# angelini/raft-simulation

Hardware: AMD Instinct MI355X
Metric: simulated node-ticks/sec (5-node Raft) (higher is better)
Workload: dtype u32; 1 GPU; C2: 65,536 5-node clusters/GPU, 10k ticks/step, no faults, no client (steady window); clusters=65536, clusters_per_gpu=65536, nodes=5, parallelism=cluster-sharded x1

## Files before the change

raft-simulation_amd/csrc/fixed_point_affine.hpp:

```cpp
#pragma once
#include <stdint.h>

#if defined(__HIPCC__)
#define FPA_FN __host__ __device__ inline __attribute__((always_inline))
#else
#define FPA_FN inline
#endif

namespace rs {
namespace fpa {

constexpr uint64_t M = 0x9E3779B97F4A7C15ull;
constexpr uint64_t M2 = M * M;
constexpr uint32_t EV_HEARTBEAT = 7, EV_APPEND_ENTRIES = 2, EV_APPEND_RESPONSE = 5;
constexpr uint32_t ROLE_LEADER = 2, ROLE_FOLLWER = 3;
constexpr uint32_t HDR_HB = EV_HEARTBEAT | ROLE_LEADER << 7;
constexpr uint32_t HDR_AR = EV_APPEND_RESPONSE | ROLE_LEADER << 7;
constexpr uint32_t HDR_AE = EV_APPEND_ENTRIES | ROLE_FOLLWER << 7;

constexpr uint64_t pow_m2(int n) {
  uint64_t x = 1;
  for (int i = 0; i < n; ++i) x *= M2;
  return x;
}
// ... 65 lines not shown
  r.z = g.a * f.z + g.z + kp * g.x;
  r.s = (uint32_t)g.a * f.s + g.s;
  return r;
}
FPA_FN Set compose(const Set& f, const Set& g, uint32_t P) {
  const uint64_t kp = (uint64_t)f.K * P;
  Set r;
  r.K = f.K + g.K;
  r.lead = compose_half(f.lead, g.lead, kp);
  r.fol = compose_half(f.fol, g.fol, kp);
  return r;
}

FPA_FN uint32_t period(int F, uint32_t d, uint32_t hb) { return 2 * d + (uint32_t)F - 1 + hb; }

template <int F>
FPA_FN Set step(const Set& c, uint32_t d, uint32_t hb) {
  return compose(c, one_round<F>(d), period(F, d, hb));
}

template <int F>
FPA_FN Set build(uint32_t d, uint32_t hb, uint32_t K) {
  const uint32_t P = period(F, d, hb);
  Set r;
  r.K = 0;
  r.lead.a = r.fol.a = 1;
  r.lead.x = r.lead.y = r.lead.z = r.fol.x = r.fol.y = r.fol.z = 0;
  r.lead.s = r.fol.s = 0;
  if (!K) return r;
  r = one_round<F>(d);
// ... 47 lines not shown
```

raft-simulation_amd/csrc/steady_kernel.hip:

```cpp
#include <hip/hip_ext.h>

#include "fixed_point_affine.hpp"
#include "tick_wave.hpp"

namespace rs {

constexpr int LANE_WG = 256;

__device__ __forceinline__ uint32_t msel(bool a, uint32_t x, uint32_t y) {
  const uint32_t m = 0u - (uint32_t)a;
  return (x & m) | (y & ~m);
}

constexpr int IMG_SLOTS = 32;
constexpr uint32_t IMG_LINE = 64 * 8 * 16;
constexpr uint32_t IMG_HALF = 2 * IMG_LINE;
constexpr uint32_t IMG_WAVE = 2 * IMG_HALF;
__device__ __forceinline__ uint32_t img_sw(uint32_t l) { return (l ^ (l >> 3)) & 7u; }
__device__ __forceinline__ uint32_t img_off(uint32_t l, uint32_t i) {
  return i < 16 ? (i >> 3) * IMG_LINE + l * 128u + 16u * ((i & 7u) ^ img_sw(l))
                : IMG_HALF + l * 256u + 16u * ((i & 15u) ^ (l & 15u));
}
template <typename T>
__device__ __forceinline__ T* lds_at(char* img, uint32_t off) {
// ... 38 lines not shown
  SetWords k[2];
};
__device__ __forceinline__ uint32_t vreg(uint32_t s) {
  uint32_t v;
  asm volatile("v_mov_b32 %0, %1" : "=v"(v) : "s"(s));
  return v;
}
__device__ __forceinline__ uint64_t vreg(uint64_t s) {
  return (uint64_t)vreg((uint32_t)(s >> 32)) << 32 | vreg((uint32_t)s);
}
__device__ __forceinline__ SetWords vreg(const fpa::Set& c, uint32_t K1) {
  return SetWords{vreg(c.lead.a), vreg(c.lead.x), vreg(c.lead.y), vreg(c.lead.z),
                  vreg(c.fol.a),  vreg(c.fol.x),  vreg(c.fol.y),  vreg(c.fol.z),
                  vreg(c.lead.s), vreg(c.fol.s),  vreg(c.K),      vreg(K1)};
}
template <int F>
__device__ __forceinline__ void band_sets(uint32_t nt, uint32_t d, uint32_t hb, BandSets* out) {
  const uint32_t P = fpa::period(F, d, hb), last = 2 * d + F - 1;
  const uint32_t K1 = nt > last ? (nt - last - 1) / P + 1 : 0;
  const fpa::Set lo = fpa::build<F>(d, hb, K1 ? K1 - 1 : 0), hi = fpa::step<F>(lo, d, hb);
  out->k[0] = vreg(lo, K1);
  out->k[1] = vreg(hi, K1);
}

template <int N>
struct FixedPoint {
  static constexpr int F = N - 1;
  uint32_t L, Lid, Lterm, Lcommit;
  uint64_t Ltr, ftr[F];
  uint32_t Ldl, fdl[F], fpend;
  uint32_t qmask, qA[F], qT[F], qa[F], qb[F];
  uint32_t rmask, resA, rT[F], rA[F], rB[F], rH[F];
  uint32_t nhb, nae, nar;

  __device__ __forceinline__ uint32_t fk(int j) const { return (uint32_t)j + ((uint32_t)j >= L ? 1u : 0u); }

  __device__ __forceinline__ void append_entries(uint32_t ta, uint32_t d, uint32_t el_base) {
#pragma unroll
    for (int j = 0; j < F; ++j) {
      ftr[j] = trace_event(ftr[j], ta, RAFT_MSG_APPEND_ENTRIES, Lid, Lterm, RAFT_FOLLWER, Lterm, 0);
      fdl[j] = ta + el_base;
      rT[j] = Lterm; rA[j] = Lcommit; rB[j] = 0; rH[j] = 1;
// ... 78 lines not shown
#pragma unroll
    for (int j = 0; j < F; ++j) {
      if (on && ((rmask >> j) & 1)) {
        uint4* dp = rp + 2 * n;
        dp[0] = make_uint4(resA, RAFT_MSG_APPEND_RESPONSE | sid(j) << 3 | rH[j] << 7, rT[j], rA[j]);
        dp[1] = make_uint4(rB[j], 0, 0, 0);
        ++n;
      }
    }
  }
};

template <int N>
struct NodeOrder {
  static constexpr int F = N - 1;
  uint32_t L, T;
  uint64_t tr[N], Ltr;
  uint32_t Ldl;
  bool qin, took;
  uint32_t qA, fdl;
  uint32_t rc, resA;
  uint32_t nhb, nae, nar;

  __device__ __forceinline__ uint32_t sid(int j) const {
    return (uint32_t)j + 1 + ((uint32_t)j >= L ? 1u : 0u);
  }
  __device__ __forceinline__ void followers(uint64_t a, uint64_t add) {
#pragma unroll
    for (int k = 0; k < N; ++k) tr[k] = tr[k] * a + add;
  }
// ... 13 lines not shown
      if ((uint32_t)j + rc >= (uint32_t)F && tau < tend) {
        Ltr = trace_event(Ltr, tau, RAFT_MSG_APPEND_RESPONSE, sid(j), T, RAFT_LEADER, T, 0);
        --rc;
        Ldl = tau + hb;
        ++nar;
      }
    }
    if (!rc) resA = INF;
  }
  __device__ __forceinline__ uint32_t term() const { return T; }
  __device__ __forceinline__ void rearmed(uint32_t v) { took = true; fdl = v; }
  __device__ __forceinline__ void heartbeat(uint32_t ta) { qin = true; qA = ta; }
  __device__ __forceinline__ bool queued() const { return rc != 0; }
};

template <typename St>
__device__ __forceinline__ void rounds(St& s, uint32_t th, uint32_t tend, uint32_t d, uint32_t hb,
                                       uint32_t el_base, const BandSets& bs) {
  constexpr int F = St::F;
  const uint32_t P = 2 * d + F - 1 + hb, last = 2 * d + F - 1, T = s.term();
  const uint32_t K = tend > th + last ? (tend - th - last - 1) / P + 1 : 0;
  const uint32_t tk = th + K * P;
  if (K) {
    const uint32_t K1 = bs.k[0].K1;
    const bool top = K == K1;
    if (!__builtin_amdgcn_ballot_w64(!top && K + 1 != K1)) {
      const SetWords sw = bs.k[top];
      const fpa::Half cl = sw.lead(), cf = sw.fol();
      s.Ltr = fpa::apply_leader<F>(cl, s.Ltr, th, T, s.L);
      s.followers(cf.a, fpa::follower_addend<F>(cf, th, T, s.L));
    } else {
      uint64_t a = trace_term(th, 7, 0, 0, RAFT_LEADER, T, 0);
#pragma unroll
      for (int j = 0; j < F; ++j)
        a = a * TRACE_M2 + trace_term(th + 2 * d + j, RAFT_MSG_APPEND_RESPONSE, s.sid(j), T,
                                      RAFT_LEADER, T, 0);
      const uint64_t da = (uint64_t)P * (TRACE_M * trace_geo<F + 1>());
      const uint64_t df = (uint64_t)P * TRACE_M;
// ... 14 lines not shown
  if (tk < tend) {
    s.Ltr = trace_event(s.Ltr, tk, 7, 0, 0, RAFT_LEADER, T, 0);
    ++s.nhb;
    s.Ldl = tk + hb;
    s.heartbeat(tk + d);
    if (tk + d < tend) {
      s.append_entries(tk + d, d, el_base);
      s.responses(tk, tend, d, hb);
    }
  }
}

template <typename St>
__device__ __forceinline__ void run_launch(St& s, uint32_t mid, uint32_t th0, uint32_t tend,
                                           uint32_t d, uint32_t hb, uint32_t el_base, uint32_t P,
                                           const BandSets& bs) {
  bool whole = true;
  if (mid == 1) {
    if (th0 + d < tend) s.append_entries(th0 + d, d, el_base);
    else whole = false;
  }
  if (mid && whole) {
    s.responses(th0, tend, d, hb);
    whole = !s.queued();
  }
  if (whole) rounds(s, mid ? th0 + P : th0, tend, d, hb, el_base, bs);
}

struct Schedule {
  uint32_t mid, th0, nxt;
  bool on;
};
template <int F>
__device__ __forceinline__ Schedule schedule(uint32_t t0, uint32_t tend, uint32_t d, uint32_t hb,
                                             uint32_t P, uint32_t Ldl, bool req, uint32_t reqA,
                                             uint32_t nres, uint32_t resA) {
  Schedule s{0, Ldl, 0, true};
  if (req) {
    s.mid = 1;
    s.th0 = reqA - d;
    s.on = reqA >= t0 && reqA >= d && Ldl == s.th0 + hb;
// ... 106 lines not shown
  };
  auto fword = [&](int f, int j, uint32_t L) {
    return msel((uint32_t)j >= L, word(f, j + 1), word(f, j));
  };
  static_assert(HF_RES_TAIL + 1 == HF_FLAGS && (HOT_CW + HF_FLAGS * N) % 4 == 0 && HOT_CW % 4 == 0,
                "the fields written: DEADLINE .. RES_TAIL, whole chunks");
  constexpr int CH_END = (int)(HOT_CW + HF_FLAGS * N) / 4;
  asm volatile("" ::"s"(nt), "s"(t0), "s"(S.dmin), "s"(S.hb), "s"(S.el_base));
  load_line(0, false);
  const bool reporter = blockIdx.x == 0 && threadIdx.x == 0;
  uint32_t prev_bails = 0;
  if (reporter) prev_bails = *S.nbail_zero;
  uint32_t nt_s = nt;
  asm volatile("" : "+s"(nt_s));
  const BandSets& bs = bs_keep[wave];
  band_sets<F>(nt_s, S.dmin, S.hb, &bs_keep[wave]);
  load_wait();
  if (reporter && prev_bails) {
    if (S.bail_report) *S.bail_report = prev_bails;
    *S.nbail_zero = 0;
  }
  static_assert(NW4 >= 8, "line 0 is read whole");
  read_chunks(0, 8);
  const uint32_t tend = t0 + nt, d = S.dmin;
  const uint32_t P = 2 * d + F - 1 + S.hb, allF = (1u << F) - 1;
  uint32_t dl = 0, nhb = 0, nae = 0, nar = 0;
  bool el = false;
  uint32_t el_to = 0;
#ifdef RS_WAVELOG
  uint64_t wl_x1 = 0, wl_x2 = 0, wl_x3 = 0, wl_lend = 0;
  uint32_t wl_cut = 0;
  asm volatile("" ::"v"(w[CL_CERT]), "v"(w[HOT_CW]));
  wl_loop = wall_clock64();
#endif

  static_assert(HOT_CW + (HF_QMETA + 1) * N <= 32 && HF_DEADLINE < HF_QMETA &&
                    HF_TRACE_LO < HF_QMETA && HF_TRACE_HI < HF_QMETA && CL_CTERM < HOT_CW,
                "every word the line-0 path reads is in line 0; REQ_ARR, RES_ARR, the flags and "
                "the term are derived (device.hpp)");
  NodeOrder<N> no;
  uint32_t lmid = 0, lth0 = 0;
  const bool cfg_ok = S.el_base >= P && S.hb >= 2 * d + F && S.Q >= (uint32_t)F;
  bool strong = active && cfg_ok && (w[CL_CERT] & 0xFFFF0000u) == CERT_STRONG &&
                (w[CL_CERT] & 0xFFFFu) < (uint32_t)N;
  {
    const uint32_t L = w[CL_CERT] & 0xFFFFu;
    no.L = L; no.T = w[CL_CTERM];
    no.Ldl = lword(HF_DEADLINE, L);
    no.Ltr = (uint64_t)lword(HF_TRACE_HI, L) << 32 | lword(HF_TRACE_LO, L);
#pragma unroll
    for (int k = 0; k < N; ++k) no.tr[k] = (uint64_t)word(HF_TRACE_HI, k) << 32 | word(HF_TRACE_LO, k);
    no.qin = no.took = false; no.qA = no.fdl = 0; no.rc = 0; no.resA = INF;
    no.nhb = no.nae = no.nar = 0;
    const uint32_t Lqm = lword(HF_QMETA, L), rsc = qm_res_cnt(Lqm);
    const uint32_t qm0 = L ? word(HF_QMETA, 0) : word(HF_QMETA, 1);
    const bool need = qm0 != 0;
    strong = strong && (qm0 & ~pack_qmeta(0, 1, 0, 0)) == 0 && Lqm == pack_qmeta(0, 0, 0, rsc) &&
             rsc <= (uint32_t)F && !(need && rsc);
#pragma unroll
    for (int k = 0; k < N; ++k) strong = strong && (L == (uint32_t)k || word(HF_QMETA, k) == qm0);
    lth0 = no.Ldl;
    if (need) {
      lmid = 1;
      lth0 = no.Ldl - S.hb;
      const uint32_t ta = lth0 + d;
      strong = strong && no.Ldl >= S.hb && ta >= t0;
      no.qin = true;
      no.qA = ta;
    } else if (rsc) {
      lmid = 2;
      const uint32_t j0 = (uint32_t)F - rsc, back = S.hb + (j0 ? 2 * d + j0 - 1 : 0u);
      lth0 = no.Ldl - back;
      const uint32_t ra = lth0 + 2 * d;
      const int64_t cut = (int64_t)t0 - (int64_t)ra;
      strong = strong && no.Ldl >= back &&
               (int64_t)j0 == (cut < 0 ? 0 : cut > F ? (int64_t)F : cut);
      no.rc = rsc;
      no.resA = ra;
    } else {
      strong = strong && no.Ldl >= t0;
    }
    const uint32_t nxt = min((lmid == 2 ? lth0 + P : lth0) + d, tend);
#pragma unroll
    for (int k = 0; k < N; ++k)
      strong = strong && (L == (uint32_t)k || word(HF_DEADLINE, k) >= nxt);
  }
  const bool line0_wave = !__builtin_amdgcn_ballot_w64(active && !strong);
  if (line0_wave) {
#ifdef RS_WAVELOG
    asm volatile("" ::"v"(no.Ltr), "v"(no.Ldl), "v"(no.tr[0]), "v"(lth0));
    wl_x1 = wl_x2 = wall_clock64();
#endif
    if (active) {
      run_launch(no, lmid, lth0, tend, d, S.hb, S.el_base, P, bs);
      nhb = no.nhb; nae = no.nae; nar = no.nar;
#ifdef RS_WAVELOG
      asm volatile("" ::"v"(no.Ltr), "v"(no.tr[0]), "v"(no.Ldl));
      wl_x3 = wall_clock64();
#endif
      const uint32_t fqm = pack_qmeta(0, no.qin ? 1u : 0u, 0, 0), Lqm = pack_qmeta(0, 0, 0, no.rc);
      const uint32_t fra = no.qin ? no.qA : INF, frt = no.qin ? no.qA : 0u;
      const uint32_t Lrt = no.rc ? no.resA : 0u;
      auto val = [&](int q) -> uint32_t {
        const int f = (q - (int)HOT_CW) / N, k = (q - (int)HOT_CW) % N;
        const bool isL = no.L == (uint32_t)k;
        switch (f) {
          case HF_DEADLINE: return isL ? no.Ldl : no.took ? no.fdl : w[q];
          case HF_TRACE_LO: return (uint32_t)(isL ? no.Ltr : no.tr[k]);
          case HF_TRACE_HI: return (uint32_t)((isL ? no.Ltr : no.tr[k]) >> 32);
          case HF_QMETA: return isL ? Lqm : fqm;
          case HF_REQ_ARR: return isL ? INF : fra;
          case HF_RES_ARR: return isL ? no.resA : INF;
          case HF_REQ_TAIL: return isL ? 0u : frt;
          default: return isL ? Lrt : 0u;
        }
      };
      auto chunk = [&](int i) {
        return make_uint4(val(4 * i), val(4 * i + 1), val(4 * i + 2), val(4 * i + 3));
      };
#pragma unroll
      for (int i = (int)HOT_CW / 4; i < (CH_END < 8 ? CH_END : 8); ++i) {
        const int q = 4 * i;
        const uint4 x = chunk(i);
        *lds_at<uint4>(img, img_off(lane, i)) = x;
        dl |= (uint32_t)(x.x != w[q] || x.y != w[q + 1] || x.z != w[q + 2] || x.w != w[q + 3]);
      }
      if (CH_END > 8 && (lmid || no.qin || no.rc)) {
        uint4* const bp = reinterpret_cast<uint4*>(S.hot + (size_t)c * HB);
#pragma unroll
        for (int i = 8; i < CH_END; ++i) bp[i] = chunk(i);
      }
    }
    if (__builtin_amdgcn_ballot_w64(active && (no.qin || no.rc))) {
      if (active && no.qin) {
#pragma unroll
        for (int k = 0; k < N; ++k) {
          if (no.L != (uint32_t)k) {
            uint4* dp = reinterpret_cast<uint4*>(qslots(S, c * N + k, 0));
            dp[0] = make_uint4(no.qA, RAFT_MSG_APPEND_ENTRIES | (no.L + 1) << 3, no.T, 0);
            dp[1] = make_uint4(0, 0, 0, 0);
          }
// ... 31 lines not shown
      Lc = lead ? (uint32_t)k : Lc;
      nlc += lead;
    }
    static_assert(HOT_CW + (HF_FLAGS + 1) * N <= 64, "the flags are in the first two lines");
    cert = active && nlc == 1 &&
           (w[CL_CERT] == (CERT_MAGIC | Lc) || w[CL_CERT] == (CERT_STRONG | Lc));
    full = IMGC > 16 && __builtin_amdgcn_ballot_w64(active && !cert) != 0;
    if (full) {
      load_half1();
      read_chunks(16, NW4);
    }
  }
  const bool vouched = cert && !full;

  FixedPoint<N> fx;
  bool lean = false;
  if (!line0_wave) {
    lean = vouched && cfg_ok;
    const uint32_t L = Lc;
    fx.L = L; fx.Lid = L + 1; fx.Lterm = lword(HF_TERM, L); fx.Lcommit = 0;
    fx.Ldl = lword(HF_DEADLINE, L);
    fx.Ltr = (uint64_t)lword(HF_TRACE_HI, L) << 32 | lword(HF_TRACE_LO, L);
    fx.qmask = fx.rmask = 0; fx.resA = INF; fx.fpend = allF; fx.nhb = fx.nae = fx.nar = 0;
    const uint32_t Lqm = lword(HF_QMETA, L);
    const uint32_t rsc = qm_res_cnt(Lqm);
    uint32_t need = 0;
#pragma unroll
    for (int j = 0; j < F; ++j) {
      fx.fdl[j] = fword(HF_DEADLINE, j, L);
      fx.ftr[j] = (uint64_t)fword(HF_TRACE_HI, j, L) << 32 | fword(HF_TRACE_LO, j, L);
      const uint32_t qm = fword(HF_QMETA, j, L);
      lean = lean && (fword(HF_FLAGS, j, L) & FL_DRAW) && ((qm >> 4) & 31) <= 1 && !qm_res_cnt(qm);
      need |= (qm_req_cnt(qm) ? 1u : 0u) << j;
      fx.qA[j] = INF; fx.qT[j] = fx.qa[j] = fx.qb[j] = 0;
      fx.rT[j] = fx.rA[j] = fx.rB[j] = fx.rH[j] = 0;
    }
    lean = lean && !qm_req_cnt(Lqm) && rsc <= (uint32_t)F && !(need && rsc) &&
           (need == 0 || need == allF);
    const uint32_t ta = fword(HF_REQ_ARR, 0, L), ra = lword(HF_RES_ARR, L);
    const Schedule sc = schedule<F>(t0, tend, d, S.hb, P, fx.Ldl, need != 0, ta, rsc, ra);
    lean = lean && sc.on;
    lmid = sc.mid;
    lth0 = sc.th0;
    if (lmid == 1) {
#pragma unroll
      for (int j = 0; j < F; ++j) {
        lean = lean && fword(HF_REQ_ARR, j, L) == ta;
        fx.qA[j] = ta; fx.qT[j] = fx.Lterm;
      }
      fx.qmask = allF;
    } else if (lmid == 2) {
      fx.rmask = allF & ~((1u << ((uint32_t)F - rsc)) - 1);
      fx.resA = ra;
#pragma unroll
      for (int j = 0; j < F; ++j) {
        fx.rT[j] = fx.Lterm; fx.rH[j] = 1;
      }
    }
#pragma unroll
    for (int j = 0; j < F; ++j) lean = lean && fx.fdl[j] >= sc.nxt;
  }
  const bool lean_wave = !line0_wave && !__builtin_amdgcn_ballot_w64(active && !lean);
  bool wb = false;
  if (lean_wave) {
#ifdef RS_WAVELOG
    asm volatile("" ::"v"(fx.Ltr), "v"(fx.fdl[0]), "v"(fx.ftr[0]), "v"(lth0));
    wl_x1 = wl_x2 = wall_clock64();
#endif
    if (active) {
      run_launch(fx, lmid, lth0, tend, d, S.hb, S.el_base, P, bs);
      nhb = fx.nhb; nae = fx.nae; nar = fx.nar;
#ifdef RS_WAVELOG
      asm volatile("" ::"v"(fx.Ltr), "v"(fx.ftr[0]), "v"(fx.Ldl));
      wl_x3 = wall_clock64();
#endif
      uint32_t v[HF_FLAGS][N];
#pragma unroll
      for (int k = 0; k < N; ++k) fx.node_words(k, v);
      auto val = [&](int q) { return v[(q - HOT_CW) / N][(q - HOT_CW) % N]; };
      auto chunk = [&](int i) {
        return make_uint4(val(4 * i), val(4 * i + 1), val(4 * i + 2), val(4 * i + 3));
      };
#pragma unroll
      for (int i = (int)HOT_CW / 4; i < CH_END; ++i) {
        const int q = 4 * i;
// ... 6 lines not shown
      *lds_at<uint4>(img, img_off(lane, CL_CERT / 4)) =
          make_uint4(w[CL_CERT - 3], w[CL_CERT - 2], fx.Lterm, cn);
      static_assert(CL_CTERM == CL_CERT - 1 && CL_CERT % 4 == 3, "one chunk");
      dl |= (uint32_t)(cn != w[CL_CERT] || fx.Lterm != w[CL_CTERM]);
    }
    fx.to_rings(S, c, active);
#ifdef RS_WAVELOG
    wl_lend = wall_clock64();
#endif
  } else if (!line0_wave) {
#ifdef RS_WAVELOG
    wl_loop = wall_clock64();
#endif
    {
      auto ifield = [&](int f, int k) { return w[HOT_CW + f * N + k]; };
      bool pat = active && w[CL_HWM_IDX] == 0 && S.Q >= 2u * F && S.el_base >= P && S.hb >= 2 * d + F;
      const uint32_t T = ifield(HF_TERM, 0);
#pragma unroll
      for (int k = 0; k < N; ++k) {
        pat = pat && ifield(HF_FLAGS, k) == 0 && ifield(HF_MASKS, k) == 0 &&
              ifield(HF_TERM, k) == T && ifield(HF_COMMIT, k) == 0 && ifield(HF_LEN, k) == 0 &&
              ifield(HF_QMETA, k) == 0 && ifield(HF_REQ_ARR, k) == INF &&
              ifield(HF_RES_ARR, k) == INF;
#pragma unroll
        for (int p = 0; p < 2 * N; ++p) pat = pat && ifield(HF_NEXT + p, k) == 0;
      }
      pat = pat && T != INF;
      uint32_t cidx = 0, t1 = INF, ntie = 0, bidx = 0;
#pragma unroll
      for (int k = 0; k < N; ++k) {
        const uint32_t dk = ifield(HF_DEADLINE, k);
// ... 44 lines not shown
          const uint32_t sid = (uint32_t)j + ((uint32_t)j >= cidx ? 2u : 1u);
          hc = trace_event(hc, (uint32_t)tau0 + j, RAFT_MSG_APPEND_RESPONSE, sid, T, RAFT_LEADER,
                           T1, 0);
        }
#pragma unroll
        for (int k = 0; k < N; ++k) {
          const bool isc = (uint32_t)k == cidx;
          uint64_t h = (uint64_t)ifield(HF_TRACE_HI, k) << 32 | ifield(HF_TRACE_LO, k);
          h = trace_event(h, t1 + d, RAFT_MSG_REQUEST_VOTE, cid, T1, RAFT_FOLLOWER, T, 0);
          h = trace_event(h, (uint32_t)tL + d, RAFT_MSG_APPEND_ENTRIES, cid, T1, RAFT_FOLLWER, T1, 0);
          h = isc ? hc : h;
          w[HOT_CW + HF_FLAGS * N + k] = isc ? pack_flags(RAFT_LEADER, 0, cid, 0, 0, 1)
                                             : pack_flags(RAFT_FOLLWER, 0, cid, 0, 0, 0) | FL_DRAW;
          w[HOT_CW + HF_MASKS * N + k] = isc ? peers << 16 : 0u;
          w[HOT_CW + HF_TERM * N + k] = T1;
          w[HOT_CW + HF_DEADLINE * N + k] = isc ? (uint32_t)tlast + S.hb
                                                : (uint32_t)tL + d + S.el_base;
          w[HOT_CW + HF_REQ_TAIL * N + k] = 0;
          w[HOT_CW + HF_RES_TAIL * N + k] = 0;
          w[HOT_CW + HF_TRACE_LO * N + k] = (uint32_t)h;
          w[HOT_CW + HF_TRACE_HI * N + k] = (uint32_t)(h >> 32);
        }
        nae = F;
        nar = F;
      } else if (pat && tie) {
        const uint32_t a = cidx, b = bidx, B = b + 1;
        const uint32_t A = cid;
        constexpr uint32_t M = (N + 1) / 2;
        uint64_t ha = 0, hbb = 0;
#pragma unroll
        for (int k = 0; k < N; ++k) {
          const uint64_t h0 = (uint64_t)ifield(HF_TRACE_HI, k) << 32 | ifield(HF_TRACE_LO, k);
// ... 19 lines not shown
        hbb = trace_event(hbb, t1 + 1, RAFT_MSG_REQUEST_VOTE, A, T1, RAFT_CANDIDATE, T1, 0);
        hbb = trace_event(hbb, t1 + 2, RAFT_MSG_VOTE_RESPONSE, A, T1, RAFT_CANDIDATE, T1, 0);
        uint32_t tb = t1 + 3, j = 0, tbae = INF, brole = RAFT_CANDIDATE, bdl = 0;
        bool bexact = false;
        for (int it = 0; it < N + 1; ++it) {
          const bool res = j < (uint32_t)N - 2, req = tbae == INF;
          if (!res && !req) break;
          if (!res && tb < tLt + 1) tb = tLt + 1;
          const bool rq = req && tb >= tLt + 1;
          bool take_req = rq;
          bexact = false;
          if (res && rq) {
            const uint4 ew = event_draw(g, B, tb, S);
            take_req = !(ew.x & 1);
            bexact = true;
            bdl = tb + S.el_base + __umulhi(ew.y, S.el_span);
          }
          if (take_req) {
            hbb = trace_event(hbb, tb, RAFT_MSG_APPEND_ENTRIES, A, T1, RAFT_FOLLWER, T1, 0);
            brole = RAFT_FOLLWER;
            tbae = tb;
          } else {
            uint32_t fid = 0, cnt = 0;
#pragma unroll
            for (int k = 0; k < N; ++k) {
              const bool other = (uint32_t)k != a && (uint32_t)k != b;
              fid = other && cnt == j ? (uint32_t)k + 1 : fid;
              cnt += other;
            }
            hbb = trace_event(hbb, tb, RAFT_MSG_VOTE_RESPONSE, fid, T, brole, T1, 0);
            ++j;
          }
          if (!bexact) bdl = tb + S.el_base;
          ++tb;
        }
        const uint32_t tbl = tb - 1;
        uint32_t ta = t1 + N + 1;
        const uint32_t fa = tLt + 2, ba = tbae + 1;
#pragma unroll
        for (int k = 0; k < N; ++k) {
          if ((uint32_t)k == a) continue;
          const bool isb = (uint32_t)k == b;
          if (isb && ba != fa) continue;
          ta = max(ta, fa);
          ha = trace_event(ha, ta, RAFT_MSG_APPEND_RESPONSE, (uint32_t)k + 1, isb ? T1 : T,
                           RAFT_LEADER, T1, 0);
          ++ta;
        }
// ... 7 lines not shown
          el = true;
          el_to = 2;
#pragma unroll
          for (int k = 0; k < N; ++k) {
            const bool isa = (uint32_t)k == a, isb = (uint32_t)k == b;
            uint64_t h = (uint64_t)ifield(HF_TRACE_HI, k) << 32 | ifield(HF_TRACE_LO, k);
            h = trace_event(h, t1 + 1, RAFT_MSG_REQUEST_VOTE, A, T1, RAFT_FOLLOWER, T, 0);
            h = trace_event(h, t1 + 2, RAFT_MSG_REQUEST_VOTE, B, T1, RAFT_FOLLOWER, T, 0);
            h = trace_event(h, tLt + 1, RAFT_MSG_APPEND_ENTRIES, A, T1, RAFT_FOLLWER, T1, 0);
            h = isa ? ha : isb ? hbb : h;
            w[HOT_CW + HF_FLAGS * N + k] =
                isa ? pack_flags(RAFT_LEADER, 0, A, 0, 0, 1)
                    : pack_flags(RAFT_FOLLWER, 0, A, 0, 0, 0) | (isb && bexact ? 0u : FL_DRAW);
            w[HOT_CW + HF_MASKS * N + k] = isa ? peers << 16 : 0u;
            w[HOT_CW + HF_TERM * N + k] = T1;
            w[HOT_CW + HF_DEADLINE * N + k] = isa ? tal + S.hb : isb ? bdl : tLt + 1 + S.el_base;
            w[HOT_CW + HF_REQ_TAIL * N + k] = 0;
            w[HOT_CW + HF_RES_TAIL * N + k] = 0;
            w[HOT_CW + HF_TRACE_LO * N + k] = (uint32_t)h;
            w[HOT_CW + HF_TRACE_HI * N + k] = (uint32_t)(h >> 32);
          }
          nae = F;
          nar = F;
        }
      }
    }
    uint32_t L = 0, nlead = 0, badn = 0;
#pragma unroll
    for (int k = 0; k < N; ++k) {
      const uint32_t f = word(HF_FLAGS, k);
      const bool lead = fl_role(f) == RAFT_LEADER;
// ... 107 lines not shown
      }
      if (!fx.rmask) fx.resA = INF;
    }
    record_bail(active && bad, t0);
    wb = active && !bad;
    bool run = wb;

    uint32_t tn = t0;
    fx.fpend = 0;
#pragma unroll
    for (int j = 0; j < F; ++j) fx.fpend |= ((ffl[j] & FL_DRAW) ? 1u : 0u) << j;
    auto draw_deadlines = [&](uint32_t due) {
#pragma unroll
      for (int j = 0; j < F; ++j) {
        if ((due >> j) & 1) {
          const uint4 wd = event_draw(g, fx.fk(j) + 1, fx.fdl[j] - S.el_base, S);
          fx.fdl[j] += __umulhi(wd.y, S.el_span);
        }
      }
      fx.fpend &= ~due;
    };
    auto next_event = [&]() {
      uint32_t m = min(fx.Ldl, fx.resA);
#pragma unroll
      for (int j = 0; j < F; ++j) m = min(m, min(fx.fdl[j], fx.qA[j]));
      return m;
    };
    auto at_fixed_point_state = [&]() {
      bool ok = Llen == 0 && !ackbad;
#pragma unroll
      for (int j = 0; j < F; ++j)
        ok = ok && fterm[j] == Lterm &&
             (ffl[j] & FL_FOLLOW) == pack_flags(RAFT_FOLLWER, 0, Lid, 0, 0, 0) &&
             fcommit[j] == flen[j] && (fmk[j] & 0xFFFFu) == 0 && nx[j] == 0 &&
             mt[j] == (int32_t)Lcommit;
      return ok;
    };
    auto at_fixed_point = [&]() {
      return S.el_base >= P && S.hb >= 2 * d + F && !fx.qmask && !fx.rmask && at_fixed_point_state();
    };
    auto fixed_point_rounds = [&](uint32_t th) { rounds(fx, th, tend, d, S.hb, S.el_base, bs); };

    bool fp = wb && S.el_base >= P && S.hb >= 2 * d + F && (vouched || at_fixed_point_state());
    const Schedule sc = schedule<F>(t0, tend, d, S.hb, P, fx.Ldl, fx.qmask != 0, fx.qA[0],
                                    __popc(fx.rmask), fx.resA);
    const uint32_t th0 = sc.th0, mid = sc.mid;
    fp = fp && sc.on;
    if (mid == 1) {
      fp = fp && fx.qmask == allF && !fx.rmask;
#pragma unroll
      for (int j = 0; j < F; ++j)
        fp = fp && fx.qA[j] == fx.qA[0] && fx.qT[j] == Lterm && fx.qa[j] == Lcommit && fx.qb[j] == 0;
    } else if (mid == 2) {
      fp = fp && fx.rmask == (allF & ~((1u << ((uint32_t)F - __popc(fx.rmask))) - 1));
#pragma unroll
      for (int j = 0; j < F; ++j)
        fp = fp && (!((fx.rmask >> j) & 1) ||
                    (fx.rT[j] == Lterm && fx.rA[j] == Lcommit && fx.rB[j] == 0 && fx.rH[j] == 1));
    }
#pragma unroll
    for (int j = 0; j < F; ++j) fp = fp && fx.fdl[j] >= sc.nxt;
    const bool vbail = vouched && wb && !fp;
    record_bail(vbail, t0);
    if (vbail) wb = run = false;
#ifdef RS_WAVELOG
    asm volatile("" ::"v"(fp), "v"(th0));
    wl_x2 = wall_clock64();
#endif
    if (fp) {
      run = false;
      run_launch(fx, mid, th0, tend, d, S.hb, S.el_base, P, bs);
    }
#ifdef RS_WAVELOG
    asm volatile("" ::"v"(fx.Ltr), "v"(fx.ftr[0]), "v"(fx.Ldl));
    wl_x3 = wall_clock64();
#endif
#ifdef RS_WAVELOG
    wl_ts = __builtin_amdgcn_s_memtime();
#endif
    bool pbail = false;
    uint32_t pbt = 0;
    for (;;) {
      record_bail(pbail, pbt);
      pbail = false;
      uint32_t t = max(tn, next_event());
      for (;;) {
// ... 53 lines not shown
      if (bail) {
        pbail = true;
        pbt = t;
        run = false;
        continue;
      }
      uint32_t tl = t;
      bool round = false;
      if (lhb) {
#pragma unroll
        for (int j = 0; j < F; ++j) {
          fx.qA[j] = t + d; fx.qT[j] = Lterm; fx.qa[j] = Lcommit;
          fx.qb[j] = nx[j] - 1 > 0 ? (uint32_t)(nx[j] - 1) : 0u;
        }
        fx.qmask = (1u << F) - 1;
        fx.Ldl = t + S.hb;
        fx.Ltr = trace_event(fx.Ltr, t, 7, 0, 0, RAFT_LEADER, Lterm, 0);
        ++fx.nhb;
        round = fx.rmask == 0 && S.hb >= 2 * d + F && S.el_base >= d + F && tend - t > d;
#pragma unroll
        for (int j = 0; j < F; ++j)
          round = round && fx.fdl[j] >= t + d && fx.qb[j] == 0 &&
                  (Lterm < fterm[j] || flen[j] <= fcommit[j]);
      }
      RS_LPH(2);
      auto append_entries = [&](uint32_t ta, uint32_t fa) {
#pragma unroll
        for (int j = 0; j < F; ++j) {
          if ((fa >> j) & 1) {
            const uint32_t mterm = fx.qT[j], rterm = fterm[j];
            const bool ok = mterm >= fterm[j];
            const uint32_t nfl2 = ok ? (ffl[j] & ~FL_FOLLOW) |
                                           pack_flags(RAFT_FOLLWER, 0, Lid, 0, 0, 0)
                                     : ffl[j];
            const uint32_t nterm = ok ? mterm : fterm[j];
            fx.ftr[j] = trace_event(fx.ftr[j], ta, RAFT_MSG_APPEND_ENTRIES, Lid, mterm, fl_role(nfl2),
                                    nterm, 0);
            if (ok) {
              fcommit[j] = flen[j];
              fmk[j] &= 0xFFFF0000u;
            }
            fterm[j] = nterm;
            ffl[j] = nfl2;
            fx.rT[j] = rterm; fx.rA[j] = ok ? fx.qa[j] : 0u; fx.rB[j] = 0; fx.rH[j] = ok;
            fx.qA[j] = INF;
            fx.fdl[j] = ta + S.el_base;
          }
        }
        fx.fpend |= fa;
        fx.qmask &= ~fa;
        fx.rmask = fa;
        fx.resA = ta + d;
        fx.nae += __popc(fa);
        tl = ta;
      };
      auto response = [&](int j, uint32_t tau, uint32_t yT, uint32_t yA, uint32_t yB, uint32_t yH,
                          int32_t& nxj, int32_t& mtj) {
        const uint32_t yid = fx.fk(j) + 1;
        if (yT > Lterm || (yH ? ackbad : ((Lmk >> (16 + yid)) & 1) == 0)) return false;
        fx.rmask &= ~(1u << j);
        Lmk |= yH << (16 + yid);
        nxj = yH ? (int32_t)yB : nxj - 1;
        mtj = yH ? (int32_t)yA : mtj;
        fx.Ldl = tau + S.hb;
        fx.Ltr = trace_event(fx.Ltr, tau, RAFT_MSG_APPEND_RESPONSE, yid, yT, RAFT_LEADER, Lterm, 0);
        ++fx.nar;
        tl = tau;
        return true;
      };
      if (round) {
        append_entries(t + d, (1u << F) - 1);
        bool go = true;
#pragma unroll
        for (int j = 0; j < F; ++j)
          go = go && t + 2 * d + j < tend &&
               response(j, t + 2 * d + j, fx.rT[j], fx.rA[j], fx.rB[j], fx.rH[j], nx[j], mt[j]);
        if (!fx.rmask) fx.resA = INF;
        if (at_fixed_point()) {
          fixed_point_rounds(t + P);
// ... 110 lines not shown
    }
    fx.to_rings(S, c, wb);
    nhb = fx.nhb; nae = fx.nae; nar = fx.nar;
  }
  {
    uint32_t* const wbase = S.hot + (size_t)cbase * HB;
    const uint32_t sub = lane >> 3, q8 = lane & 7;
#pragma unroll
    for (int ln = 0; ln < IMGC / 8; ++ln) {
      const uint64_t bal = __builtin_amdgcn_ballot_w64((dl >> ln) & 1);
      if (!bal) continue;
      uint4 xs[8];
#pragma unroll
      for (int gq = 0; gq < 8; ++gq)
        xs[gq] = *lds_at<const uint4>(img, img_off(8 * gq + sub, 8 * ln + q8));
#pragma unroll
      for (int gq = 0; gq < 8; ++gq) {
        const uint32_t cc = 8 * gq + sub;
        if ((bal >> cc) & 1) {
          typedef uint32_t v4u __attribute__((ext_vector_type(4)));
          const v4u xv = {xs[gq].x, xs[gq].y, xs[gq].z, xs[gq].w};
          uint32_t* const dst = wbase + cc * HB + 4 * (8 * ln + q8);
          asm volatile("global_store_dwordx4 %0, %1, off sc1" : : "v"(dst), "v"(xv) : "memory");
        }
      }
    }
  }
#ifdef RS_WAVELOG
  {
    const uint64_t wl_end = wall_clock64();
    const uint32_t wl_events = nhb + nae + nar;
    const uint32_t emax = ~wave_min(~wl_events), emin = wave_min(wl_events);
    if (lane == 0 && S.wavelog) {
      uint32_t hw, xcc;
      asm volatile("s_getreg_b32 %0, hwreg(HW_REG_HW_ID)" : "=s"(hw));
// ... 2 lines not shown
      rec[0] = make_uint4((uint32_t)wl_start, (uint32_t)(wl_start >> 32), (uint32_t)wl_end,
                          (uint32_t)(wl_end >> 32));
      rec[1] = make_uint4(wl_trips, hw, xcc, wl_first);
      rec[2] = make_uint4((uint32_t)(wl_loop - wl_start), (uint32_t)(wl_lend - wl_start), emin, emax);
      rec[3] = make_uint4(wl_ph[0], wl_ph[1], wl_ph[2], wl_ph[3]);
      rec[4] = make_uint4(wl_ph[4], 0, 0, 0);
      rec[5] = make_uint4((uint32_t)(wl_x1 - wl_start), (uint32_t)(wl_x2 - wl_start),
                          (uint32_t)(wl_x3 - wl_start), wl_cut);
    }
  }
#endif
  {
    const uint32_t h = wave_sum(nhb), a = wave_sum(nae), r = wave_sum(nar);
    unsigned long long* const ctr =
        S.ctr + (size_t)((blockIdx.x * 4 + wave) % CTR_COPIES) * CTR_STRIDE;
    if (lane < 5) {
      const uint32_t msgs = (uint32_t)F * h + a;
      const int idx = lane == 0 ? RAFT_CTR_EV_HEARTBEAT : lane == 1 ? RAFT_CTR_EV_AE
                    : lane == 2 ? RAFT_CTR_EV_AR : lane == 3 ? RAFT_CTR_SENT : RAFT_CTR_DELIVERED;
      const uint32_t v = lane == 0 ? h : lane == 1 ? a : lane == 2 ? r : msgs;
      if (v) atomicAdd(&ctr[idx], (unsigned long long)v);
    }
    if (__builtin_amdgcn_ballot_w64(el)) {
      const uint32_t ne = wave_sum(el ? 1u : 0u), nt = wave_sum(el_to);
      if (lane < 6) {
        const int idx = lane == 0 ? RAFT_CTR_EV_TIMEOUT : lane == 1 ? RAFT_CTR_EV_RV
                      : lane == 2 ? RAFT_CTR_EV_VR : lane == 3 ? RAFT_CTR_LEADERS
                      : lane == 4 ? RAFT_CTR_SENT : RAFT_CTR_DELIVERED;
        const uint32_t v = lane == 0 ? nt : lane == 3 ? ne : lane <= 2 ? (uint32_t)F * nt
                                                                   : (uint32_t)F * (2 * nt + ne);
        atomicAdd(&ctr[idx], (unsigned long long)v);
      }
    }
  }
  if (nbw) {
    if (lane == 0) atomicAdd(S.nbail, nbw);
// ... 47 lines not shown
```

Measured before the change: 529300 billion node-ticks/s.

## Derive per-cluster round counts from a launch-wide band instead of per-lane division

Precomputes a launch-wide band (round count, remainder, ticks) once per wave, parks it in lanes of a VGPR, and lets the strong-path NodeOrder rounds pick K, tick offset and the composed affine set from the start-tick offset, with no per-lane division or ballot branching. The strong-certificate setup is rewritten branch-free with mask selects. The dirty-line flag is derived from event counts instead of comparing every chunk word. A fully-active writeback uses an unconditional store loop, and the counter atomics use a packed index table. This trims per-cluster ALU work and divergence on the hot steady path, at the cost of relying on every cluster's start tick lying within one period of t0 (newly added to the strong check) and on event counts tracking changed state.

```diff
diff --git a/raft-simulation_amd/csrc/fixed_point_affine.hpp b/raft-simulation_amd/csrc/fixed_point_affine.hpp
--- a/raft-simulation_amd/csrc/fixed_point_affine.hpp
+++ b/raft-simulation_amd/csrc/fixed_point_affine.hpp
@@ -103,6 +103,29 @@
 
 FPA_FN uint32_t period(int F, uint32_t d, uint32_t hb) { return 2 * d + (uint32_t)F - 1 + hb; }
 
+struct Band {
+  uint32_t K1, rho, K1P;
+};
+FPA_FN Band band(int F, uint32_t d, uint32_t hb, uint32_t nt) {
+  const uint32_t P = period(F, d, hb), last = 2 * d + (uint32_t)F - 1;
+  Band b;
+  if (nt > last) {
+    const uint32_t R = nt - last - 1, q = R / P;
+    b.K1 = q + 1;
+    b.rho = R - q * P;
+    b.K1P = b.K1 * P;
+  } else {
+    b.K1 = 0;
+    b.rho = 0xFFFFFFFFu;
+    b.K1P = 0;
+  }
+  return b;
+}
+FPA_FN uint32_t band_rounds(const Band& b, uint32_t delta) { return b.K1 - (uint32_t)(delta > b.rho); }
+FPA_FN uint32_t band_ticks(const Band& b, uint32_t P, uint32_t delta) {
+  return b.K1P - (delta > b.rho ? P : 0u);
+}
+
 template <int F>
 FPA_FN Set step(const Set& c, uint32_t d, uint32_t hb) {
   return compose(c, one_round<F>(d), period(F, d, hb));
diff --git a/raft-simulation_amd/csrc/steady_kernel.hip b/raft-simulation_amd/csrc/steady_kernel.hip
--- a/raft-simulation_amd/csrc/steady_kernel.hip
+++ b/raft-simulation_amd/csrc/steady_kernel.hip
@@ -76,18 +76,26 @@
                   vreg(c.fol.a),  vreg(c.fol.x),  vreg(c.fol.y),  vreg(c.fol.z),
                   vreg(c.lead.s), vreg(c.fol.s),  vreg(c.K),      vreg(K1)};
 }
+template <int I>
+__device__ __forceinline__ void park_lane(uint32_t& park, uint32_t v) {
+  asm volatile("v_writelane_b32 %0, %1, %2"
+               : "+v"(park)
+               : "s"(__builtin_amdgcn_readfirstlane(v)), "n"(I));
+}
 template <int F>
-__device__ __forceinline__ void band_sets(uint32_t nt, uint32_t d, uint32_t hb, BandSets* out) {
-  const uint32_t P = fpa::period(F, d, hb), last = 2 * d + F - 1;
-  const uint32_t K1 = nt > last ? (nt - last - 1) / P + 1 : 0;
+__device__ __forceinline__ fpa::Band band_sets(uint32_t nt, uint32_t d, uint32_t hb, BandSets* out) {
+  const fpa::Band b = fpa::band(F, d, hb, nt);
+  const uint32_t K1 = b.K1;
   const fpa::Set lo = fpa::build<F>(d, hb, K1 ? K1 - 1 : 0), hi = fpa::step<F>(lo, d, hb);
   out->k[0] = vreg(lo, K1);
   out->k[1] = vreg(hi, K1);
+  return b;
 }
 
 template <int N>
 struct FixedPoint {
   static constexpr int F = N - 1;
+  static constexpr bool IN_BAND = false;
   uint32_t L, Lid, Lterm, Lcommit;
   uint64_t Ltr, ftr[F];
   uint32_t Ldl, fdl[F], fpend;
@@ -196,6 +204,7 @@
 template <int N>
 struct NodeOrder {
   static constexpr int F = N - 1;
+  static constexpr bool IN_BAND = true;
   uint32_t L, T;
   uint64_t tr[N], Ltr;
   uint32_t Ldl;
@@ -239,14 +248,36 @@
   __device__ __forceinline__ bool queued() const { return rc != 0; }
 };
 
+struct LaunchBand {
+  uint32_t t0;
+  fpa::Band b;
+};
 template <typename St>
 __device__ __forceinline__ void rounds(St& s, uint32_t th, uint32_t tend, uint32_t d, uint32_t hb,
-                                       uint32_t el_base, const BandSets& bs) {
+                                       uint32_t el_base, const BandSets& bs, const LaunchBand& lb) {
   constexpr int F = St::F;
   const uint32_t P = 2 * d + F - 1 + hb, last = 2 * d + F - 1, T = s.term();
-  const uint32_t K = tend > th + last ? (tend - th - last - 1) / P + 1 : 0;
-  const uint32_t tk = th + K * P;
-  if (K) {
+  uint32_t K, tk;
+  if constexpr (St::IN_BAND) {
+    const uint32_t delta = th - lb.t0;
+    K = fpa::band_rounds(lb.b, delta);
+    tk = th + fpa::band_ticks(lb.b, P, delta);
+    const SetWords sw = bs.k[(delta <= lb.b.rho) & (lb.b.K1 != 0)];
+    const fpa::Half cl = sw.lead(), cf = sw.fol();
+    s.Ltr = fpa::apply_leader<F>(cl, s.Ltr, th, T, s.L);
+    s.followers(cf.a, fpa::follower_addend<F>(cf, th, T, s.L));
+    if (K) {
+      s.rearmed(tk - P + d + el_base);
+      s.Ldl = tk;
+      s.nhb += K;
+      s.nae += F * K;
+      s.nar += F * K;
+    }
+  } else {
+    K = tend > th + last ? (tend - th - last - 1) / P + 1 : 0;
+    tk = th + K * P;
+  }
+  if (!St::IN_BAND && K) {
     const uint32_t K1 = bs.k[0].K1;
     const bool top = K == K1;
     if (!__builtin_amdgcn_ballot_w64(!top && K + 1 != K1)) {
@@ -291,7 +322,7 @@
 template <typename St>
 __device__ __forceinline__ void run_launch(St& s, uint32_t mid, uint32_t th0, uint32_t tend,
                                            uint32_t d, uint32_t hb, uint32_t el_base, uint32_t P,
-                                           const BandSets& bs) {
+                                           const BandSets& bs, const LaunchBand& lb) {
   bool whole = true;
   if (mid == 1) {
     if (th0 + d < tend) s.append_entries(th0 + d, d, el_base);
@@ -301,7 +332,7 @@
     s.responses(th0, tend, d, hb);
     whole = !s.queued();
   }
-  if (whole) rounds(s, mid ? th0 + P : th0, tend, d, hb, el_base, bs);
+  if (whole) rounds(s, mid ? th0 + P : th0, tend, d, hb, el_base, bs, lb);
 }
 
 struct Schedule {
@@ -438,16 +469,28 @@
   uint32_t nt_s = nt;
   asm volatile("" : "+s"(nt_s));
   const BandSets& bs = bs_keep[wave];
-  band_sets<F>(nt_s, S.dmin, S.hb, &bs_keep[wave]);
+  uint32_t park = 0;
+  {
+    const fpa::Band b = band_sets<F>(nt_s, S.dmin, S.hb, &bs_keep[wave]);
+    park_lane<0>(park, b.K1);
+    park_lane<1>(park, b.rho);
+    park_lane<2>(park, b.K1P);
+  }
   load_wait();
+  asm volatile("" : "+v"(park));
+  auto parked_band = [&]() {
+    return fpa::Band{(uint32_t)__builtin_amdgcn_readlane(park, 0),
+                     (uint32_t)__builtin_amdgcn_readlane(park, 1),
+                     (uint32_t)__builtin_amdgcn_readlane(park, 2)};
+  };
   if (reporter && prev_bails) {
     if (S.bail_report) *S.bail_report = prev_bails;
     *S.nbail_zero = 0;
   }
   static_assert(NW4 >= 8, "line 0 is read whole");
   read_chunks(0, 8);
-  const uint32_t tend = t0 + nt, d = S.dmin;
-  const uint32_t P = 2 * d + F - 1 + S.hb, allF = (1u << F) - 1;
+  const uint32_t tend = t0 + nt, d = S.dmin, hb = S.hb, el_base = S.el_base;
+  const uint32_t P = 2 * d + F - 1 + hb, allF = (1u << F) - 1;
   uint32_t dl = 0, nhb = 0, nae = 0, nar = 0;
   bool el = false;
   uint32_t el_to = 0;
@@ -464,9 +507,9 @@
                 "the term are derived (device.hpp)");
   NodeOrder<N> no;
   uint32_t lmid = 0, lth0 = 0;
-  const bool cfg_ok = S.el_base >= P && S.hb >= 2 * d + F && S.Q >= (uint32_t)F;
-  bool strong = active && cfg_ok && (w[CL_CERT] & 0xFFFF0000u) == CERT_STRONG &&
-                (w[CL_CERT] & 0xFFFFu) < (uint32_t)N;
+  const bool cfg_ok = el_base >= P && hb >= 2 * d + F && S.Q >= (uint32_t)F;
+  bool strong = active & cfg_ok & ((w[CL_CERT] & 0xFFFF0000u) == CERT_STRONG) &
+                ((w[CL_CERT] & 0xFFFFu) < (uint32_t)N);
   {
     const uint32_t L = w[CL_CERT] & 0xFFFFu;
     no.L = L; no.T = w[CL_CTERM];
@@ -474,40 +517,36 @@
     no.Ltr = (uint64_t)lword(HF_TRACE_HI, L) << 32 | lword(HF_TRACE_LO, L);
 #pragma unroll
     for (int k = 0; k < N; ++k) no.tr[k] = (uint64_t)word(HF_TRACE_HI, k) << 32 | word(HF_TRACE_LO, k);
-    no.qin = no.took = false; no.qA = no.fdl = 0; no.rc = 0; no.resA = INF;
+    no.took = false; no.fdl = 0;
     no.nhb = no.nae = no.nar = 0;
     const uint32_t Lqm = lword(HF_QMETA, L), rsc = qm_res_cnt(Lqm);
     const uint32_t qm0 = L ? word(HF_QMETA, 0) : word(HF_QMETA, 1);
     const bool need = qm0 != 0;
-    strong = strong && (qm0 & ~pack_qmeta(0, 1, 0, 0)) == 0 && Lqm == pack_qmeta(0, 0, 0, rsc) &&
-             rsc <= (uint32_t)F && !(need && rsc);
-#pragma unroll
-    for (int k = 0; k < N; ++k) strong = strong && (L == (uint32_t)k || word(HF_QMETA, k) == qm0);
-    lth0 = no.Ldl;
-    if (need) {
-      lmid = 1;
-      lth0 = no.Ldl - S.hb;
-      const uint32_t ta = lth0 + d;
-      strong = strong && no.Ldl >= S.hb && ta >= t0;
-      no.qin = true;
-      no.qA = ta;
-    } else if (rsc) {
-      lmid = 2;
-      const uint32_t j0 = (uint32_t)F - rsc, back = S.hb + (j0 ? 2 * d + j0 - 1 : 0u);
-      lth0 = no.Ldl - back;
-      const uint32_t ra = lth0 + 2 * d;
-      const int64_t cut = (int64_t)t0 - (int64_t)ra;
-      strong = strong && no.Ldl >= back &&
-               (int64_t)j0 == (cut < 0 ? 0 : cut > F ? (int64_t)F : cut);
-      no.rc = rsc;
-      no.resA = ra;
-    } else {
-      strong = strong && no.Ldl >= t0;
-    }
-    const uint32_t nxt = min((lmid == 2 ? lth0 + P : lth0) + d, tend);
+    const bool cutr = !need & (rsc != 0);
+    const uint32_t one_req = pack_qmeta(0, 1, 0, 0), only_res = pack_qmeta(0, 0, 0, rsc);
+    strong = strong & ((qm0 & ~one_req) == 0) & (Lqm == only_res) & (rsc <= (uint32_t)F) &
+             !(need & (rsc != 0));
+#pragma unroll
+    for (int k = 0; k < N; ++k) strong = strong & ((L == (uint32_t)k) | (word(HF_QMETA, k) == qm0));
+    const uint32_t j0 = (uint32_t)F - rsc;
+    const uint32_t back = msel(need | cutr, hb + msel(cutr & (j0 != 0), 2 * d + j0 - 1, 0u), 0u);
+    lmid = msel(need, 1u, msel(cutr, 2u, 0u));
+    lth0 = no.Ldl - back;
+    const uint32_t ta = lth0 + d, ra = lth0 + 2 * d;
+    const int64_t cut = (int64_t)t0 - (int64_t)ra;
+    const bool on_need = ta >= t0;
+    const bool on_cut = (int64_t)j0 == (cut < 0 ? 0 : cut > F ? (int64_t)F : cut);
+    const bool on_none = no.Ldl >= t0;
+    strong = strong & (no.Ldl >= back) & (need ? on_need : cutr ? on_cut : on_none);
+    no.qin = need;
+    no.qA = msel(need, ta, 0u);
+    no.rc = msel(cutr, rsc, 0u);
+    no.resA = msel(cutr, ra, INF);
+    const uint32_t nxt = min(msel(cutr, lth0 + P, lth0) + d, tend);
 #pragma unroll
     for (int k = 0; k < N; ++k)
-      strong = strong && (L == (uint32_t)k || word(HF_DEADLINE, k) >= nxt);
+      strong = strong & ((L == (uint32_t)k) | (word(HF_DEADLINE, k) >= nxt));
+    strong = strong & (msel(lmid != 0, lth0 + P, lth0) - t0 < P);
   }
   const bool line0_wave = !__builtin_amdgcn_ballot_w64(active && !strong);
   if (line0_wave) {
@@ -516,7 +555,8 @@
     wl_x1 = wl_x2 = wall_clock64();
 #endif
     if (active) {
-      run_launch(no, lmid, lth0, tend, d, S.hb, S.el_base, P, bs);
+      const LaunchBand lb{t0, parked_band()};
+      run_launch(no, lmid, lth0, tend, d, hb, el_base, P, bs, lb);
       nhb = no.nhb; nae = no.nae; nar = no.nar;
 #ifdef RS_WAVELOG
       asm volatile("" ::"v"(no.Ltr), "v"(no.tr[0]), "v"(no.Ldl));
@@ -543,12 +583,9 @@
         return make_uint4(val(4 * i), val(4 * i + 1), val(4 * i + 2), val(4 * i + 3));
       };
 #pragma unroll
-      for (int i = (int)HOT_CW / 4; i < (CH_END < 8 ? CH_END : 8); ++i) {
-        const int q = 4 * i;
-        const uint4 x = chunk(i);
-        *lds_at<uint4>(img, img_off(lane, i)) = x;
-        dl |= (uint32_t)(x.x != w[q] || x.y != w[q + 1] || x.z != w[q + 2] || x.w != w[q + 3]);
-      }
+      for (int i = (int)HOT_CW / 4; i < (CH_END < 8 ? CH_END : 8); ++i)
+        *lds_at<uint4>(img, img_off(lane, i)) = chunk(i);
+      dl = (nhb | nae | nar) != 0;
       if (CH_END > 8 && (lmid || no.qin || no.rc)) {
         uint4* const bp = reinterpret_cast<uint4*>(S.hot + (size_t)c * HB);
 #pragma unroll
@@ -610,6 +647,7 @@
   const bool vouched = cert && !full;
 
   FixedPoint<N> fx;
+  const LaunchBand no_band{t0, fpa::Band{0, 0, 0}};
   bool lean = false;
   if (!line0_wave) {
     lean = vouched && cfg_ok;
@@ -634,7 +672,7 @@
     lean = lean && !qm_req_cnt(Lqm) && rsc <= (uint32_t)F && !(need && rsc) &&
            (need == 0 || need == allF);
     const uint32_t ta = fword(HF_REQ_ARR, 0, L), ra = lword(HF_RES_ARR, L);
-    const Schedule sc = schedule<F>(t0, tend, d, S.hb, P, fx.Ldl, need != 0, ta, rsc, ra);
+    const Schedule sc = schedule<F>(t0, tend, d, hb, P, fx.Ldl, need != 0, ta, rsc, ra);
     lean = lean && sc.on;
     lmid = sc.mid;
     lth0 = sc.th0;
@@ -664,7 +702,7 @@
     wl_x1 = wl_x2 = wall_clock64();
 #endif
     if (active) {
-      run_launch(fx, lmid, lth0, tend, d, S.hb, S.el_base, P, bs);
+      run_launch(fx, lmid, lth0, tend, d, hb, el_base, P, bs, no_band);
       nhb = fx.nhb; nae = fx.nae; nar = fx.nar;
 #ifdef RS_WAVELOG
       asm volatile("" ::"v"(fx.Ltr), "v"(fx.ftr[0]), "v"(fx.Ldl));
@@ -701,7 +739,7 @@
 #endif
     {
       auto ifield = [&](int f, int k) { return w[HOT_CW + f * N + k]; };
-      bool pat = active && w[CL_HWM_IDX] == 0 && S.Q >= 2u * F && S.el_base >= P && S.hb >= 2 * d + F;
+      bool pat = active && w[CL_HWM_IDX] == 0 && S.Q >= 2u * F && el_base >= P && hb >= 2 * d + F;
       const uint32_t T = ifield(HF_TERM, 0);
 #pragma unroll
       for (int k = 0; k < N; ++k) {
@@ -776,8 +814,8 @@
                                              : pack_flags(RAFT_FOLLWER, 0, cid, 0, 0, 0) | FL_DRAW;
           w[HOT_CW + HF_MASKS * N + k] = isc ? peers << 16 : 0u;
           w[HOT_CW + HF_TERM * N + k] = T1;
-          w[HOT_CW + HF_DEADLINE * N + k] = isc ? (uint32_t)tlast + S.hb
-                                                : (uint32_t)tL + d + S.el_base;
+          w[HOT_CW + HF_DEADLINE * N + k] = isc ? (uint32_t)tlast + hb
+                                                : (uint32_t)tL + d + el_base;
           w[HOT_CW + HF_REQ_TAIL * N + k] = 0;
           w[HOT_CW + HF_RES_TAIL * N + k] = 0;
           w[HOT_CW + HF_TRACE_LO * N + k] = (uint32_t)h;
@@ -827,7 +865,7 @@
             const uint4 ew = event_draw(g, B, tb, S);
             take_req = !(ew.x & 1);
             bexact = true;
-            bdl = tb + S.el_base + __umulhi(ew.y, S.el_span);
+            bdl = tb + el_base + __umulhi(ew.y, S.el_span);
           }
           if (take_req) {
             hbb = trace_event(hbb, tb, RAFT_MSG_APPEND_ENTRIES, A, T1, RAFT_FOLLWER, T1, 0);
@@ -844,7 +882,7 @@
             hbb = trace_event(hbb, tb, RAFT_MSG_VOTE_RESPONSE, fid, T, brole, T1, 0);
             ++j;
           }
-          if (!bexact) bdl = tb + S.el_base;
+          if (!bexact) bdl = tb + el_base;
           ++tb;
         }
         const uint32_t tbl = tb - 1;
@@ -882,7 +920,7 @@
                     : pack_flags(RAFT_FOLLWER, 0, A, 0, 0, 0) | (isb && bexact ? 0u : FL_DRAW);
             w[HOT_CW + HF_MASKS * N + k] = isa ? peers << 16 : 0u;
             w[HOT_CW + HF_TERM * N + k] = T1;
-            w[HOT_CW + HF_DEADLINE * N + k] = isa ? tal + S.hb : isb ? bdl : tLt + 1 + S.el_base;
+            w[HOT_CW + HF_DEADLINE * N + k] = isa ? tal + hb : isb ? bdl : tLt + 1 + el_base;
             w[HOT_CW + HF_REQ_TAIL * N + k] = 0;
             w[HOT_CW + HF_RES_TAIL * N + k] = 0;
             w[HOT_CW + HF_TRACE_LO * N + k] = (uint32_t)h;
@@ -1020,7 +1058,7 @@
 #pragma unroll
       for (int j = 0; j < F; ++j) {
         if ((due >> j) & 1) {
-          const uint4 wd = event_draw(g, fx.fk(j) + 1, fx.fdl[j] - S.el_base, S);
+          const uint4 wd = event_draw(g, fx.fk(j) + 1, fx.fdl[j] - el_base, S);
           fx.fdl[j] += __umulhi(wd.y, S.el_span);
         }
       }
@@ -1043,12 +1081,12 @@
       return ok;
     };
     auto at_fixed_point = [&]() {
-      return S.el_base >= P && S.hb >= 2 * d + F && !fx.qmask && !fx.rmask && at_fixed_point_state();
+      return el_base >= P && hb >= 2 * d + F && !fx.qmask && !fx.rmask && at_fixed_point_state();
     };
-    auto fixed_point_rounds = [&](uint32_t th) { rounds(fx, th, tend, d, S.hb, S.el_base, bs); };
-
-    bool fp = wb && S.el_base >= P && S.hb >= 2 * d + F && (vouched || at_fixed_point_state());
-    const Schedule sc = schedule<F>(t0, tend, d, S.hb, P, fx.Ldl, fx.qmask != 0, fx.qA[0],
+    auto fixed_point_rounds = [&](uint32_t th) { rounds(fx, th, tend, d, hb, el_base, bs, no_band); };
+
+    bool fp = wb && el_base >= P && hb >= 2 * d + F && (vouched || at_fixed_point_state());
+    const Schedule sc = schedule<F>(t0, tend, d, hb, P, fx.Ldl, fx.qmask != 0, fx.qA[0],
                                     __popc(fx.rmask), fx.resA);
     const uint32_t th0 = sc.th0, mid = sc.mid;
     fp = fp && sc.on;
@@ -1075,7 +1113,7 @@
 #endif
     if (fp) {
       run = false;
-      run_launch(fx, mid, th0, tend, d, S.hb, S.el_base, P, bs);
+      run_launch(fx, mid, th0, tend, d, hb, el_base, P, bs, no_band);
     }
 #ifdef RS_WAVELOG
     asm volatile("" ::"v"(fx.Ltr), "v"(fx.ftr[0]), "v"(fx.Ldl));
@@ -1159,10 +1197,10 @@
           fx.qb[j] = nx[j] - 1 > 0 ? (uint32_t)(nx[j] - 1) : 0u;
         }
         fx.qmask = (1u << F) - 1;
-        fx.Ldl = t + S.hb;
+        fx.Ldl = t + hb;
         fx.Ltr = trace_event(fx.Ltr, t, 7, 0, 0, RAFT_LEADER, Lterm, 0);
         ++fx.nhb;
-        round = fx.rmask == 0 && S.hb >= 2 * d + F && S.el_base >= d + F && tend - t > d;
+        round = fx.rmask == 0 && hb >= 2 * d + F && el_base >= d + F && tend - t > d;
 #pragma unroll
         for (int j = 0; j < F; ++j)
           round = round && fx.fdl[j] >= t + d && fx.qb[j] == 0 &&
@@ -1189,7 +1227,7 @@
             ffl[j] = nfl2;
             fx.rT[j] = rterm; fx.rA[j] = ok ? fx.qa[j] : 0u; fx.rB[j] = 0; fx.rH[j] = ok;
             fx.qA[j] = INF;
-            fx.fdl[j] = ta + S.el_base;
+            fx.fdl[j] = ta + el_base;
           }
         }
         fx.fpend |= fa;
@@ -1207,7 +1245,7 @@
         Lmk |= yH << (16 + yid);
         nxj = yH ? (int32_t)yB : nxj - 1;
         mtj = yH ? (int32_t)yA : mtj;
-        fx.Ldl = tau + S.hb;
+        fx.Ldl = tau + hb;
         fx.Ltr = trace_event(fx.Ltr, tau, RAFT_MSG_APPEND_RESPONSE, yid, yT, RAFT_LEADER, Lterm, 0);
         ++fx.nar;
         tl = tau;
@@ -1348,11 +1386,21 @@
 #pragma unroll
       for (int gq = 0; gq < 8; ++gq)
         xs[gq] = *lds_at<const uint4>(img, img_off(8 * gq + sub, 8 * ln + q8));
+      typedef uint32_t v4u __attribute__((ext_vector_type(4)));
+      if (bal == ~0ull) {
+        uint32_t* const dst0 = wbase + sub * HB + 4 * (8 * ln + q8);
+#pragma unroll
+        for (int gq = 0; gq < 8; ++gq) {
+          const v4u xv = {xs[gq].x, xs[gq].y, xs[gq].z, xs[gq].w};
+          uint32_t* const dst = dst0 + (size_t)(8 * gq) * HB;
+          asm volatile("global_store_dwordx4 %0, %1, off sc1" : : "v"(dst), "v"(xv) : "memory");
+        }
+        continue;
+      }
 #pragma unroll
       for (int gq = 0; gq < 8; ++gq) {
         const uint32_t cc = 8 * gq + sub;
         if ((bal >> cc) & 1) {
-          typedef uint32_t v4u __attribute__((ext_vector_type(4)));
           const v4u xv = {xs[gq].x, xs[gq].y, xs[gq].z, xs[gq].w};
           uint32_t* const dst = wbase + cc * HB + 4 * (8 * ln + q8);
           asm volatile("global_store_dwordx4 %0, %1, off sc1" : : "v"(dst), "v"(xv) : "memory");
@@ -1385,12 +1433,14 @@
     const uint32_t h = wave_sum(nhb), a = wave_sum(nae), r = wave_sum(nar);
     unsigned long long* const ctr =
         S.ctr + (size_t)((blockIdx.x * 4 + wave) % CTR_COPIES) * CTR_STRIDE;
-    if (lane < 5) {
+    {
+      constexpr uint32_t IDX = RAFT_CTR_EV_HEARTBEAT | RAFT_CTR_EV_AE << 4 | RAFT_CTR_EV_AR << 8 |
+                               RAFT_CTR_SENT << 12 | RAFT_CTR_DELIVERED << 16;
+      static_assert(RAFT_CTR_DELIVERED < 16, "a nibble per index");
       const uint32_t msgs = (uint32_t)F * h + a;
-      const int idx = lane == 0 ? RAFT_CTR_EV_HEARTBEAT : lane == 1 ? RAFT_CTR_EV_AE
-                    : lane == 2 ? RAFT_CTR_EV_AR : lane == 3 ? RAFT_CTR_SENT : RAFT_CTR_DELIVERED;
-      const uint32_t v = lane == 0 ? h : lane == 1 ? a : lane == 2 ? r : msgs;
-      if (v) atomicAdd(&ctr[idx], (unsigned long long)v);
+      const uint32_t idx = (IDX >> (4 * (lane & 7))) & 15u;
+      const uint32_t v = msel(lane == 0, h, msel(lane == 1, a, msel(lane == 2, r, msgs)));
+      if (lane < 5 && v) atomicAdd(&ctr[idx], (unsigned long long)v);
     }
     if (__builtin_amdgcn_ballot_w64(el)) {
       const uint32_t ne = wave_sum(el ? 1u : 0u), nt = wave_sum(el_to);
```

Measured after the change: 573300 billion node-ticks/s (median of 6 runs). 1.08x the previous value.
